# AiX-im/Sample-based-GNN

Hardware: AMD Instinct MI355X
Metric: sampled-edges/sec + epoch time, 2-hop GCN on Reddit-shaped graph @1/2/4/8 GPUs (higher is better)
Workload: dtype fp32 (GEMM inputs fp32, split exactly into three bf16 pieces in the kernels, 6 bf16 MFMA products, fp32 accumulate; aggregation fp32)

## Files before the change

### sample-based-gnn_amd/csrc/gemmx3.hip

```cpp
#include "mfma_lds.hpp"
#include <type_traits>

namespace nts_hip {


__device__ __forceinline__ f32x16 x3_mfma6(const bf16x8 (&a)[3], const bf16x8 (&b)[3], f32x16 acc) {
  acc = __builtin_amdgcn_mfma_f32_32x32x16_bf16(a[2], b[0], acc, 0, 0, 0);
  acc = __builtin_amdgcn_mfma_f32_32x32x16_bf16(a[1], b[1], acc, 0, 0, 0);
  acc = __builtin_amdgcn_mfma_f32_32x32x16_bf16(a[0], b[2], acc, 0, 0, 0);
  acc = __builtin_amdgcn_mfma_f32_32x32x16_bf16(a[1], b[0], acc, 0, 0, 0);
  acc = __builtin_amdgcn_mfma_f32_32x32x16_bf16(a[0], b[1], acc, 0, 0, 0);
  acc = __builtin_amdgcn_mfma_f32_32x32x16_bf16(a[0], b[0], acc, 0, 0, 0);
  return acc;
}

constexpr int kX3Threads = 512;
constexpr int kX3BRaw = 16 * 512;
constexpr int kX3BPl = 16 * 256;



template <int TPW, int PR, bool BM = false>
__global__ __launch_bounds__(kX3Threads, 1) void k_x3_tn(int M, int K, const float* __restrict__ X,
                                                        uint64_t ldx, const uint32_t* __restrict__ amap,
                                                        const float* __restrict__ B, uint64_t ldb,
                                                        float* __restrict__ C, uint64_t ldc, int kchunk,
                                                        uint64_t split_stride, int nnb,
                                                        const float* __restrict__ Xm, uint64_t ldxm,
                                                        float bscale) {
  static_assert(2 * PR <= 6, "X DMA pieces per wave and step");
  extern __shared__ __attribute__((aligned(16))) char x3tn[];
  const int Kp = (M + 31) / 32 * 32, RB = 4 * Kp, RW = Kp;
  const int xstage = 16 * RB;
  char* const sx = x3tn;
  char* const sbr = sx + 3 * xstage;
  char* const sbp = sbr + 2 * kX3BRaw;
  char* const sbm = sbp + 6 * kX3BPl;
  uint32_t* const sid = reinterpret_cast<uint32_t*>(sbm + (BM ? 2 * kX3BRaw : 0));
  const int tid = threadIdx.x, lane = tid & 63;
  const int wv = __builtin_amdgcn_readfirstlane(tid >> 6);
  const int nb = blockIdx.x % nnb, split = blockIdx.x / nnb;
  const int n0 = nb * 128;
  const int kbeg = split * kchunk, kend = min(K, kbeg + kchunk), klast = kend - kbeg - 1;
  if (klast < 0) return;
  const int nsteps = (kend - kbeg + 15) / 16;
  for (int k = tid; k < 16 * (nsteps + 3); k += kX3Threads)
    sid[k] = amap ? amap[kbeg + min(k, klast)] : (uint32_t)(kbeg + min(k, klast));
  __syncthreads();
  const uint32_t lsx = lds_addr(sx), lsbr = lds_addr(sbr), lsbm = lds_addr(sbm);
  auto ids_read = [&](int s) { return *reinterpret_cast<const uint2*>(sid + 16 * s + 2 * wv); };
  auto ids_uni = [&](uint2 u) {
    return make_uint2(__builtin_amdgcn_readfirstlane(u.x), __builtin_amdgcn_readfirstlane(u.y));
  };
  auto issue_x1 = [&](int s, uint2 id, int q) {
    const int row = 2 * wv + q / PR, part = q % PR;
    const int off = 1024 * part + 16 * lane;
    const char* src = reinterpret_cast<const char*>(X + (uint64_t)(q < PR ? id.x : id.y) * ldx) + off;
    const uint32_t dst = __builtin_amdgcn_readfirstlane(lsx + (s % 3) * xstage + row * RB + 1024 * part);
    if (off < RB) glds16(src, dst);
  };
  auto issue_b = [&](int s) {
    const int row = 2 * wv + (lane >> 5);
    const int k = kbeg + min(16 * s + row, klast);
    glds16(B + (uint64_t)k * ldb + n0 + 4 * (lane & 31), lsbr + (s & 1) * kX3BRaw + 1024 * wv);
    if constexpr (BM)
      glds16(Xm + (uint64_t)k * ldxm + n0 + 4 * (lane & 31), lsbm + (s & 1) * kX3BRaw + 1024 * wv);
  };
  const int sr = tid >> 5, sc = 4 * (tid & 31);
  const int soff = tr_off(sr, sc / 8) + 8 * ((sc / 4) & 1);
  auto splitb_read = [&](int s) {
    float4 v = *reinterpret_cast<const float4*>(sbr + (s & 1) * kX3BRaw + 512 * sr + 4 * sc);
    if constexpr (BM) {
      const float4 m = *reinterpret_cast<const float4*>(sbm + (s & 1) * kX3BRaw + 512 * sr + 4 * sc);
      v.x = m.x > 0.f ? v.x * bscale : 0.f;
      v.y = m.y > 0.f ? v.y * bscale : 0.f;
      v.z = m.z > 0.f ? v.z * bscale : 0.f;
      v.w = m.w > 0.f ? v.w * bscale : 0.f;
    }
    return v;
  };
  auto splitb_write = [&](int s, float4 v) {
    const bool ok = 16 * s + sr <= klast;
    uint32_t q0[2], q1[2], q2[2];
    split3_pair(ok ? v.x : 0.f, ok ? v.y : 0.f, q0[0], q1[0], q2[0]);
    split3_pair(ok ? v.z : 0.f, ok ? v.w : 0.f, q0[1], q1[1], q2[1]);
    char* dst = sbp + (s & 1) * 3 * kX3BPl + soff;
    *reinterpret_cast<uint2*>(dst) = make_uint2(q0[0], q0[1]);
    *reinterpret_cast<uint2*>(dst + kX3BPl) = make_uint2(q1[0], q1[1]);
    *reinterpret_cast<uint2*>(dst + 2 * kX3BPl) = make_uint2(q2[0], q2[1]);
  };
  const int wn = wv & 1, wm = wv >> 1;
  const int T32 = (M + 31) / 32;
  const int m_lo = wm * T32 / 4, nmt = (wm + 1) * T32 / 4 - m_lo;
  const int c = lane & 31, h = lane >> 5;
  const int half = (lane >> 4) & 1, tq = (lane & 15) >> 2, tp = lane & 3;
  int boff[2][2];
#pragma unroll
  for (int nt = 0; nt < 2; ++nt) {
    const int ch = (2 * (64 * wn + 32 * nt + 16 * half + 4 * tp)) / 16;
    boff[nt][0] = tr_off(8 * h + tq, ch) + 8 * (tp & 1);
    boff[nt][1] = tr_off(8 * h + tq + 4, ch) + 8 * (tp & 1);
  }
  int xcol[TPW];
#pragma unroll
  for (int t = 0; t < TPW; ++t) xcol[t] = 32 * max(0, min(m_lo + min(t, nmt - 1), T32 - 1)) + 8 * h * RW + c;
  f32x16 acc[TPW][2];
#pragma unroll
  for (int t = 0; t < TPW; ++t)
#pragma unroll
    for (int nt = 0; nt < 2; ++nt)
#pragma unroll
      for (int v = 0; v < 16; ++v) acc[t][nt][v] = 0.f;
  issue_b(0);
  asm volatile("s_waitcnt vmcnt(0)" ::: "memory");
  raw_barrier();
  splitb_write(0, splitb_read(0));
  issue_b(1);
  {
    const uint2 i0 = ids_uni(ids_read(0)), i1 = ids_uni(ids_read(1));
#pragma unroll
    for (int q = 0; q < 2 * PR; ++q) issue_x1(0, i0, q);
#pragma unroll
    for (int q = 0; q < 2 * PR; ++q) issue_x1(1, i1, q);
  }
  uint2 idn = ids_uni(ids_read(2));
  for (int s = 0; s < nsteps; ++s) {
    asm volatile("s_waitcnt vmcnt(0)" ::: "memory");
    raw_barrier();
    issue_b(s + 2);
    const char* pl = sbp + (s & 1) * 3 * kX3BPl;
    bf16x8 bq[2][3];
#pragma unroll
    for (int nt = 0; nt < 2; ++nt)
#pragma unroll
      for (int p = 0; p < 3; ++p) {
        const s16x4 lo = __builtin_amdgcn_ds_read_tr16_b64_v4i16((lds_s16x4*)(pl + p * kX3BPl + boff[nt][0]));
        const s16x4 hi = __builtin_amdgcn_ds_read_tr16_b64_v4i16((lds_s16x4*)(pl + p * kX3BPl + boff[nt][1]));
        const s16x8 w = {lo[0], lo[1], lo[2], lo[3], hi[0], hi[1], hi[2], hi[3]};
        bq[nt][p] = __builtin_bit_cast(bf16x8, w);
      }
    const float* xs = reinterpret_cast<const float*>(sx + (s % 3) * xstage);
    float xr[2][8];
    uint32_t ap[2][3][4];
    auto rd = [&](int t, int j) { return xs[xcol[t] + j * RW]; };
    auto sp = [&](int t, int jp) {
      split3_pair(xr[t & 1][2 * jp], xr[t & 1][2 * jp + 1], ap[t & 1][0][jp], ap[t & 1][1][jp],
                ap[t & 1][2][jp]);
    };
#pragma unroll
    for (int j = 0; j < 8; ++j) xr[0][j] = rd(0, j);
    if constexpr (TPW > 1) {
#pragma unroll
      for (int j = 0; j < 8; ++j) xr[1][j] = rd(1, j);
    }
#pragma unroll
    for (int jp = 0; jp < 4; ++jp) sp(0, jp);
    const uint2 idx = idn;
    float4 bv = make_float4(0.f, 0.f, 0.f, 0.f);
    uint2 idr = make_uint2(0u, 0u);
#pragma unroll
    for (int t = 0; t < TPW; ++t) {
      bf16x8 a[3];
#pragma unroll
      for (int p = 0; p < 3; ++p)
        a[p] = __builtin_bit_cast(bf16x8, (u32x4){ap[t & 1][p][0], ap[t & 1][p][1], ap[t & 1][p][2], ap[t & 1][p][3]});
#pragma unroll
      for (int k = 0; k < 12; ++k) {
        __builtin_amdgcn_sched_barrier(0);
        {
          const int nt = k & 1, pr = k >> 1;
          const int pa = pr == 0 ? 2 : pr == 1 ? 1 : pr == 2 ? 0 : pr == 3 ? 1 : 0;
          const int pb = pr == 0 ? 0 : pr == 1 ? 1 : pr == 2 ? 2 : pr == 3 ? 0 : pr == 4 ? 1 : 0;
          acc[t][nt] = __builtin_amdgcn_mfma_f32_32x32x16_bf16(a[pa], bq[nt][pb], acc[t][nt], 0, 0, 0);
        }
        if (t + 2 < TPW && k < 8) xr[t & 1][k] = rd(t + 2, k);
        if (t + 1 < TPW && (k == 3 || k == 5 || k == 7 || k == 9)) sp(t + 1, (k - 3) / 2);
        if (t == 0 && (k & 1) && k / 2 < 2 * PR) issue_x1(s + 2, idx, k / 2);
        constexpr int tB = TPW >= 2 ? 1 : 0, kBr = TPW >= 2 ? 1 : 5, kBw = TPW >= 2 ? 8 : 9;
        constexpr int tI = TPW >= 3 ? 2 : 0, kIr = TPW >= 3 ? 1 : 6, kIw = TPW >= 3 ? 10 : 11;
        if (t == tB && k == kBr) bv = splitb_read(s + 1);
        if (t == tB && k == kBw) splitb_write(s + 1, bv);
        if (t == tI && k == kIr) idr = ids_read(s + 3);
        if (t == tI && k == kIw) idn = ids_uni(idr);
      }
      __builtin_amdgcn_sched_barrier(0);
    }
  }
  asm volatile("s_waitcnt vmcnt(0)" ::: "memory");
  raw_barrier();
  float* Cb = C + (uint64_t)split * split_stride;
#pragma unroll
  for (int nt = 0; nt < 2; ++nt) {
    const int col = n0 + 64 * wn + 32 * nt + c;
#pragma unroll
    for (int t = 0; t < TPW; ++t) {
      if (t >= nmt) continue;
#pragma unroll
      for (int v = 0; v < 16; ++v) {
        const int row = 32 * (m_lo + t) + 8 * (v / 4) + 4 * h + (v % 4);
        if (row < M) Cb[(uint64_t)row * ldc + col] = acc[t][nt][v];
      }
    }
  }
}

constexpr int kX3NnImg = 8 * 3 * 1024;
constexpr int kX3NnAWave = 2 * 2048;
constexpr int kX3NnA = 8 * kX3NnAWave;
constexpr int kX3NnLds = 2 * kX3NnImg + 3 * kX3NnA;
struct X3Epi {
  uint32_t keep_threshold = 0;
  float scale = 1.f;
  uint64_t seed = 0, offset = 0;
};


template <bool EPI>
__global__ __launch_bounds__(kX3Threads, 1) void k_x3_nn(int M, int N, int K, const float* __restrict__ X,
                                                        uint64_t ldx, const uint32_t* __restrict__ amap,
                                                        const char* __restrict__ bimg,
                                                        float* __restrict__ C, uint64_t ldc, int rounds,
                                                        X3Epi ep) {
  extern __shared__ __attribute__((aligned(16))) char x3nn[];
  char* const sb = x3nn;
  char* const sa = x3nn + 2 * kX3NnImg;
  const int tid = threadIdx.x, lane = tid & 63;
  const int wv = __builtin_amdgcn_readfirstlane(tid >> 6);
  const int i = lane & 15, q = lane >> 4;
  const int nb = blockIdx.y, n0 = nb * 128;
  const int T = (M + 15) / 16;
  const int64_t Wn = (int64_t)gridDim.x * 8, gw = (int64_t)blockIdx.x * 8 + wv;
  const int t_lo = (int)(gw * T / Wn), t_hi = (int)((gw + 1) * T / Wn);
  const int nsteps = (K + 31) / 32;
  const size_t bstride = (size_t)gridDim.y * kX3NnImg;
  const uint32_t lsb = lds_addr(sb), lsa = lds_addr(sa);
  const char* bsrc = bimg + (size_t)nb * kX3NnImg + wv * 1024 + 16 * lane;
  const int gr = (lane >> 1) & 15, gpo = 8 * (lane >> 5) + 4 * (lane & 1);
  const float* arow[2];
  auto set_rows = [&](int rd) {
#pragma unroll
    for (int rt = 0; rt < 2; ++rt) {
      const int t = min(t_lo + 2 * rd + rt, T - 1);
      const int64_t row = (int64_t)t * 16 + gr;
      const uint64_t rr = (uint64_t)(row < M ? row : M - 1);
      arow[rt] = X + (amap ? (uint64_t)amap[rr] : rr) * ldx + gpo;
    }
  };
  auto issue_b = [&](int s) {
    const uint32_t dst = lsb + (s & 1) * kX3NnImg + wv * 1024;
    const char* src = bsrc + (size_t)s * bstride;
#pragma unroll
    for (int p = 0; p < 3; ++p) glds16(src + 8192 * p, dst + 8192 * p);
  };
  auto issue_a = [&](int s) {
    const uint32_t dst = lsa + (s % 3) * kX3NnA + wv * kX3NnAWave;
#pragma unroll
    for (int rt = 0; rt < 2; ++rt)
#pragma unroll
      for (int h = 0; h < 2; ++h) glds16(arow[rt] + 32 * s + 16 * h, dst + rt * 2048 + h * 1024);
  };
  f32x4 acc[2][8];
  float xr[2][8];
  uint32_t ap[2][2][3][4];
  auto read_a = [&](int s, int rt) {
    typedef float f4v __attribute__((ext_vector_type(4)));
    const char* as = sa + (s % 3) * kX3NnA + wv * kX3NnAWave + 32 * (i + 16 * q) + rt * 2048;
    const f4v u = *reinterpret_cast<const f4v*>(as);
    const f4v v = *reinterpret_cast<const f4v*>(as + 16);
    const float x[8] = {u[0], u[1], u[2], u[3], v[0], v[1], v[2], v[3]};
#pragma unroll
    for (int j = 0; j < 8; ++j) xr[rt][j] = x[j];
    if (32 * s + 32 > K) {
#pragma unroll
      for (int j = 0; j < 8; ++j) xr[rt][j] = 32 * s + 8 * q + j < K ? x[j] : 0.f;
    }
  };
  auto split_a = [&](auto par, int rt, int jp) {
    constexpr int P = decltype(par)::value;
    split3_pair(xr[rt][2 * jp], xr[rt][2 * jp + 1], ap[P][rt][0][jp], ap[P][rt][1][jp], ap[P][rt][2][jp]);
  };
  auto step = [&](int s, auto par, auto ntc) {
    constexpr int P = decltype(par)::value, NT = decltype(ntc)::value;
    if (s > 0) {
      asm volatile("s_waitcnt vmcnt(0)" ::: "memory");
      raw_barrier();
      if (s + 1 < nsteps) issue_b(s + 1);
      if (s + 2 < nsteps) issue_a(s + 2);
    }
    const char* img = sb + (s & 1) * kX3NnImg;
    auto getb = [&](int ct, int p) {
      return *reinterpret_cast<const bf16x8*>(img + ct * 3072 + p * 1024 + 16 * lane);
    };
    bf16x8 bf[2][3];
#pragma unroll
    for (int p = 0; p < 3; ++p) bf[0][p] = getb(0, p);
    bf16x8 a[2][3];
#pragma unroll
    for (int rt = 0; rt < NT; ++rt)
#pragma unroll
      for (int p = 0; p < 3; ++p)
        a[rt][p] = __builtin_bit_cast(bf16x8, (u32x4){ap[P][rt][p][0], ap[P][rt][p][1], ap[P][rt][p][2], ap[P][rt][p][3]});
#pragma unroll
    for (int ct = 0; ct < 8; ++ct) {
#pragma unroll
      for (int k = 0; k < 6 * NT; ++k) {
        __builtin_amdgcn_sched_barrier(0);
        {
          const int rt = NT == 2 ? (k & 1) : 0, pr = NT == 2 ? (k >> 1) : k;
          const int pa = pr == 0 ? 2 : pr == 1 ? 1 : pr == 2 ? 0 : pr == 3 ? 1 : 0;
          const int pb = pr == 0 ? 0 : pr == 1 ? 1 : pr == 2 ? 2 : pr == 3 ? 0 : pr == 4 ? 1 : 0;
          if constexpr (EPI)
            acc[rt][ct] = __builtin_amdgcn_mfma_f32_16x16x32_bf16(a[rt][pa], bf[ct & 1][pb], acc[rt][ct], 0, 0, 0);
          else
            acc[rt][ct] = __builtin_amdgcn_mfma_f32_16x16x32_bf16(bf[ct & 1][pb], a[rt][pa], acc[rt][ct], 0, 0, 0);
        }
        if (ct + 1 < 8 && (k == 0 || k == 2 || k == 4)) bf[(ct + 1) & 1][k / 2] = getb(ct + 1, k / 2);
        if (ct == 4 && k == 0) asm volatile("s_waitcnt vmcnt(0)" ::: "memory");
        if (ct == 4 && k == 1) read_a(s + 1, 0);
        if constexpr (NT == 2) {
          if (ct == 4 && k == 3) read_a(s + 1, 1);
          if ((ct == 5 || ct == 6) && k % 3 == 1) split_a(std::integral_constant<int, 1 - P>{}, ct - 5, k / 3);
        } else {
          if (ct == 5 && (k & 1)) split_a(std::integral_constant<int, 1 - P>{}, 0, k >> 1);
          if (ct == 6 && k == 1) split_a(std::integral_constant<int, 1 - P>{}, 0, 3);
        }
      }
      __builtin_amdgcn_sched_barrier(0);
    }
  };
  auto round_steps = [&](auto ntc) {
    constexpr int NT = decltype(ntc)::value;
    issue_b(0);
    issue_a(0);
    if (nsteps > 1) issue_a(1);
    asm volatile("s_waitcnt vmcnt(0)" ::: "memory");
    raw_barrier();
    if (nsteps > 1) issue_b(1);
    if (nsteps > 2) issue_a(2);
#pragma unroll
    for (int rt = 0; rt < NT; ++rt) read_a(0, rt);
#pragma unroll
    for (int rt = 0; rt < NT; ++rt)
#pragma unroll
      for (int jp = 0; jp < 4; ++jp) split_a(std::integral_constant<int, 0>{}, rt, jp);
    for (int s = 0; s < nsteps; s += 2) {
      step(s, std::integral_constant<int, 0>{}, ntc);
      if (s + 1 < nsteps) step(s + 1, std::integral_constant<int, 1>{}, ntc);
    }
  };
  for (int rd = 0; rd < rounds; ++rd) {
    const int nt = min(2, max(0, t_hi - (t_lo + 2 * rd)));
    set_rows(rd);
#pragma unroll
    for (int rt = 0; rt < 2; ++rt)
#pragma unroll
      for (int ct = 0; ct < 8; ++ct) acc[rt][ct] = f32x4{0.f, 0.f, 0.f, 0.f};
    if (nt == 2) round_steps(std::integral_constant<int, 2>{});
    else round_steps(std::integral_constant<int, 1>{});
    raw_barrier();
    if constexpr (!EPI) {
#pragma unroll
      for (int rt = 0; rt < 2; ++rt) {
        if (rt >= nt) continue;
        const int64_t row = (int64_t)(t_lo + 2 * rd + rt) * 16 + i;
        if (row >= M) continue;
#pragma unroll
        for (int ct = 0; ct < 8; ++ct) {
          const int col = n0 + 16 * ct + 4 * q;
          if (col >= N) continue;
          float* dst = C + (uint64_t)row * ldc + col;
          if (ldc % 4 == 0 && (uintptr_t)C % 16 == 0)
            *reinterpret_cast<f32x4*>(dst) = acc[rt][ct];
          else
#pragma unroll
            for (int v = 0; v < 4; ++v) dst[v] = acc[rt][ct][v];
        }
      }
      continue;
    }
#pragma unroll
    for (int rt = 0; rt < 2; ++rt) {
      if (rt >= nt) continue;
      const int64_t r4 = (int64_t)(t_lo + 2 * rd + rt) * 16 + 4 * q;
#pragma unroll
      for (int ct = 0; ct < 8; ++ct) {
        const uint32_t col = (uint32_t)(n0 + 16 * ct + i);
        if ((int)col >= N) continue;
        float o[4] = {acc[rt][ct][0], acc[rt][ct][1], acc[rt][ct][2], acc[rt][ct][3]};
        if constexpr (EPI) {
          const uint4 rnd = dropout_words((uint64_t)r4, col, ep.seed, ep.offset);
          const uint32_t wd[4] = {rnd.x, rnd.y, rnd.z, rnd.w};
#pragma unroll
          for (int v = 0; v < 4; ++v)
            o[v] = (dropout_bits(wd[v], col) >= ep.keep_threshold && o[v] > 0.f) ? o[v] * ep.scale : 0.f;
        }
#pragma unroll
        for (int v = 0; v < 4; ++v)
          if (r4 + v < M) C[(uint64_t)(r4 + v) * ldc + col] = o[v];
      }
    }
  }
}

constexpr int kX3N7Threads = 256;
constexpr int kX3N7RT = 7;
constexpr int kX3N7Lds = 3 * kX3NnImg;
__device__ constexpr int kX3N7Pb[kX3N7RT] = {0, 1, 2, 0, 1, 2, 1};

template <int B, int E, class F>
__device__ __forceinline__ void x3_sfor(F&& f) {
  if constexpr (B < E) {
    f(std::integral_constant<int, B>{});
    x3_sfor<B + 1, E>(f);
  }
}

template <int O>
__device__ __forceinline__ void x3_split_op(const float (&x)[8], float (&r)[8], float (&f)[8],
                                            uint32_t (&p)[3][4]) {
  auto pk = [](float a, float b) {
    return __builtin_bit_cast(uint32_t, __builtin_convertvector((f32x2){a, b}, bf16x2));
  };
  if constexpr (O < 4) {
    p[0][O] = pk(x[2 * O], x[2 * O + 1]);
  } else if constexpr (O < 12) {
    constexpr int e = O - 4;
    f[e] = __uint_as_float((e & 1) ? (p[0][e / 2] & 0xffff0000u) : (p[0][e / 2] << 16));
  } else if constexpr (O < 20) {
    r[O - 12] = x[O - 12] - f[O - 12];
  } else if constexpr (O < 24) {
    p[1][O - 20] = pk(r[2 * (O - 20)], r[2 * (O - 20) + 1]);
  } else if constexpr (O < 32) {
    constexpr int e = O - 24;
    f[e] = __uint_as_float((e & 1) ? (p[1][e / 2] & 0xffff0000u) : (p[1][e / 2] << 16));
  } else if constexpr (O < 40) {
    r[O - 32] = r[O - 32] - f[O - 32];
  } else if constexpr (O < 44) {
    p[2][O - 40] = pk(r[2 * (O - 40)], r[2 * (O - 40) + 1]);
  }
}

constexpr int kX3N7Bq = 1;
template <int RT, bool EPI = false>
__global__ __launch_bounds__(kX3N7Threads, 1) void k_x3_nn7(int M, int N, int K, const float* __restrict__ X,
                                                           uint64_t ldx, const uint32_t* __restrict__ amap,
                                                           const char* __restrict__ bimg, float* __restrict__ C,
                                                           uint64_t ldc, int rounds, X3Epi ep) {
  static_assert(RT == kX3N7RT, "the W piece schedule is written for 7 tiles");
  extern __shared__ __attribute__((aligned(16))) char x3n7[];
  const int tid = threadIdx.x, lane = tid & 63;
  const int wv = __builtin_amdgcn_readfirstlane(tid >> 6);
  const int i = lane & 15, q = lane >> 4;
  const int nb = blockIdx.y, n0 = nb * 128;
  const int T = (M + 15) / 16;
  const int64_t Wn = (int64_t)gridDim.x * 4, gw = (int64_t)blockIdx.x * 4 + wv;
  const int t_lo = (int)(gw * T / Wn), t_hi = (int)((gw + 1) * T / Wn);
  const int nsteps = (K + 31) / 32;
  const uint64_t bstride = (uint64_t)gridDim.y * kX3NnImg;
  const uint32_t lsw = lds_addr(x3n7) + 6144 * wv;
  const char* bsrc = bimg + (size_t)nb * kX3NnImg + 6144 * wv + 16 * lane;
  auto row_id = [&](int rd, int rt) -> uint32_t {
    int t = min(t_lo + RT * rd + rt, max(t_hi, t_lo + 1) - 1);
    t = min(t, T - 1);
    int64_t r = (int64_t)t * 16 + i;
    if (r >= M) r = M - 1;
    return amap ? amap[r] : (uint32_t)r;
  };
  const float* ptr[RT];
  uint32_t nid[RT];
#pragma unroll
  for (int rt = 0; rt < RT; ++rt) ptr[rt] = X + (uint64_t)row_id(0, rt) * ldx + 8 * q;
#pragma unroll
  for (int rt = 0; rt < RT; ++rt) nid[rt] = row_id(1, rt);
  f32x4 wst[6];
  char* const wdst = x3n7 + 6144 * wv + 16 * lane;
  auto load_w = [&](int s, auto pc) {
    constexpr int piece = decltype(pc)::value;
    wst[piece] = *reinterpret_cast<const f32x4*>(bsrc + (size_t)s * bstride + 1024 * piece);
  };
  const uint32_t wdst_l = lds_addr(wdst);
  auto store_w = [&](int buf, auto pc) {
    constexpr int piece = decltype(pc)::value;
    const uint32_t addr = wdst_l + buf * kX3NnImg;
    const f32x4 v = wst[piece];
    asm volatile("ds_write_b128 %0, %1 offset:%2" ::"v"(addr), "v"(v), "n"(1024 * piece) : "memory");
  };
  float4 raw[RT][2];
  auto load_a = [&](int rt, int s) {
    const float* p = ptr[rt] + 32 * s;
    raw[rt][0] = *reinterpret_cast<const float4*>(p);
    raw[rt][1] = *reinterpret_cast<const float4*>(p + 4);
  };
  f32x4 acc[RT][8];
#pragma unroll
  for (int rt = 0; rt < RT; ++rt)
#pragma unroll
    for (int ct = 0; ct < 8; ++ct) acc[rt][ct] = f32x4{0.f, 0.f, 0.f, 0.f};
  uint32_t pcs[3][3][4];
  constexpr int NB = kX3N7Bq + 1;
  bf16x8 bq[NB][3];
  float sr[8], sf[8];
  auto read_b = [&](int buf, int ct, int p) {
    return *reinterpret_cast<const bf16x8*>(x3n7 + buf * kX3NnImg + ct * 3072 + p * 1024 + 16 * lane);
  };
  auto mask_k = [&](float (&x)[8], int s) {
    if (32 * s + 32 > K) {
#pragma unroll
      for (int j = 0; j < 8; ++j) x[j] = 32 * s + 8 * q + j < K ? x[j] : 0.f;
    }
  };
  auto raw8 = [&](int rt, float (&x)[8]) {
    x[0] = raw[rt][0].x; x[1] = raw[rt][0].y; x[2] = raw[rt][0].z; x[3] = raw[rt][0].w;
    x[4] = raw[rt][1].x; x[5] = raw[rt][1].y; x[6] = raw[rt][1].z; x[7] = raw[rt][1].w;
  };
  x3_sfor<0, 6>([&](auto pc) {
    load_w(0, pc);
    store_w(0, pc);
  });
#pragma unroll
  for (int rt = 0; rt < RT; ++rt) load_a(rt, 0);
  asm volatile("s_waitcnt vmcnt(0)" ::: "memory");
  raw_barrier();
  {
    float x[8];
    raw8(0, x);
    mask_k(x, 0);
#pragma unroll
    for (int j = 0; j < 4; ++j) split3_pair(x[2 * j], x[2 * j + 1], pcs[0][0][j], pcs[0][1][j], pcs[0][2][j]);
  }
  load_a(0, 1);
#pragma unroll
  for (int c = 0; c < kX3N7Bq; ++c)
#pragma unroll
    for (int p = 0; p < 3; ++p) bq[c][p] = read_b(0, c, p);
  int wb = 0;
  for (int rd = 0; rd < rounds; ++rd) {
  for (int s = 0; s < nsteps; ++s) {
    int s1 = s + 1, rd1 = rd;
    if (s1 == nsteps) { s1 = 0; ++rd1; }
    int s2 = s1 + 1, rd2 = rd1;
    if (s2 == nsteps) { s2 = 0; ++rd2; }
    const int wb1 = wb == 2 ? 0 : wb + 1;
    x3_sfor<0, RT>([&](auto rtc) {
      constexpr int rt = decltype(rtc)::value;
      constexpr int cur = kX3N7Pb[rt], nxt = kX3N7Pb[rt + 1 < RT ? rt + 1 : 0];
      bf16x8 a[3];
#pragma unroll
      for (int p = 0; p < 3; ++p)
        a[p] = __builtin_bit_cast(bf16x8, (u32x4){pcs[cur][p][0], pcs[cur][p][1], pcs[cur][p][2], pcs[cur][p][3]});
      constexpr int srt = rt + 1 < RT ? rt + 1 : 0;
      const int ss = rt + 1 < RT ? s : s1;
      float x[8];
      if constexpr (rt + 1 == RT) {
        x3_sfor<0, 6>([&](auto pc) { store_w(wb1, pc); });
        asm volatile("s_waitcnt lgkmcnt(0)" ::: "memory");
        raw_barrier();
      }
      __builtin_amdgcn_sched_barrier(0);
      raw8(srt, x);
      mask_k(x, ss);
      x3_sfor<0, 48>([&](auto kc) {
        constexpr int k = decltype(kc)::value;
        constexpr int ct = k / 6, pr = k % 6;
        __builtin_amdgcn_sched_barrier(0);
        {
          constexpr int pa = pr == 0 ? 2 : pr == 1 ? 1 : pr == 2 ? 0 : pr == 3 ? 1 : 0;
          constexpr int pb = pr == 0 ? 0 : pr == 1 ? 1 : pr == 2 ? 2 : pr == 3 ? 0 : pr == 4 ? 1 : 0;
          if constexpr (EPI)
            acc[rt][ct] = __builtin_amdgcn_mfma_f32_16x16x32_bf16(a[pa], bq[ct % NB][pb], acc[rt][ct], 0, 0, 0);
          else
            acc[rt][ct] = __builtin_amdgcn_mfma_f32_16x16x32_bf16(bq[ct % NB][pb], a[pa], acc[rt][ct], 0, 0, 0);
        }
        if constexpr (pr < 3) {
          constexpr int cn = ct + kX3N7Bq;
          if constexpr (cn < 8) bq[cn % NB][pr] = read_b(wb, cn, pr);
          else if constexpr (rt + 1 < RT) bq[(cn - 8) % NB][pr] = read_b(wb, cn - 8, pr);
          else bq[(cn - 8) % NB][pr] = read_b(wb1, cn - 8, pr);
        }
        if constexpr (k >= 1 && k <= 44) x3_split_op<k - 1>(x, sr, sf, pcs[nxt]);
        if constexpr (rt + 1 < RT) {
          if constexpr (rt == 0 && k >= 2 && k < 8)
            load_w(s1, std::integral_constant<int, (k >= 2 && k < 8 ? k - 2 : 0)>{});
        }
        if constexpr (k == 22) {
          if constexpr (rt + 1 < RT) {
            if (s1 == 0 && rd1 < rounds) ptr[srt] = X + (uint64_t)nid[srt] * ldx + 8 * q;
            load_a(srt, s1);
          } else {
            if (s2 == 0 && rd2 < rounds) ptr[0] = X + (uint64_t)nid[0] * ldx + 8 * q;
            load_a(0, s2);
          }
        }
      });
      __builtin_amdgcn_sched_barrier(0);
    });
    wb = wb1;
  }
    {
      x3_sfor<0, RT>([&](auto rtc) {
        constexpr int rt = decltype(rtc)::value;
        const int t = t_lo + RT * rd + rt;
        if constexpr (!EPI) {
          const int64_t row = (int64_t)t * 16 + i;
          if (t < t_hi && row < M) {
#pragma unroll
            for (int ct = 0; ct < 8; ++ct) {
              const int col = n0 + 16 * ct + 4 * q;
              if (col < N) *reinterpret_cast<f32x4*>(C + (uint64_t)row * ldc + col) = acc[rt][ct];
            }
          }
        } else if (t < t_hi) {
          const int64_t r4 = (int64_t)t * 16 + 4 * q;
          x3_sfor<0, 8>([&](auto ctc) {
            constexpr int ct = decltype(ctc)::value;
            const uint32_t col = (uint32_t)(n0 + 16 * ct + i);
            if ((int)col < N) {
              const uint4 rnd = dropout_words((uint64_t)r4, col, ep.seed, ep.offset);
              const uint32_t wd[4] = {rnd.x, rnd.y, rnd.z, rnd.w};
              x3_sfor<0, 4>([&](auto vc) {
                constexpr int v = decltype(vc)::value;
                const float o = acc[rt][ct][v];
                if (r4 + v < M)
                  C[(uint64_t)(r4 + v) * ldc + col] =
                      (dropout_bits(wd[v], col) >= ep.keep_threshold && o > 0.f) ? o * ep.scale : 0.f;
              });
            }
          });
        }
#pragma unroll
        for (int ct = 0; ct < 8; ++ct) acc[rt][ct] = f32x4{0.f, 0.f, 0.f, 0.f};
      });
#pragma unroll
      for (int rt = 0; rt < RT; ++rt) nid[rt] = row_id(rd + 2, rt);
    }
  }
  asm volatile("s_waitcnt vmcnt(0)" ::: "memory");
}


bool x3_tn_ok(int M, int N, int K, const float* A, uint64_t lda, const float* B, uint64_t ldb,
              const float* Xm, uint64_t ldxm) {
  const int Kp = (M + 31) / 32 * 32;
  const int lds = 3 * 16 * 4 * Kp + 2 * kX3BRaw + 6 * kX3BPl + (Xm ? 2 * kX3BRaw : 0) + 4 * 16 * 3 +
                  4 * 256;
  return M >= 32 && lds <= 160 * 1024 && N % 128 == 0 && K >= 256 && lda >= (uint64_t)Kp && lda % 4 == 0 &&
         (uintptr_t)A % 16 == 0 && ldb % 4 == 0 && (uintptr_t)B % 16 == 0 &&
         (!Xm || (ldxm % 4 == 0 && (uintptr_t)Xm % 16 == 0));
}

int x3_tn(nts_hip_ctx* ctx, int M, int N, int K, const float* A, uint64_t lda, const uint32_t* amap,
          const float* B, uint64_t ldb, float* C, uint64_t ldc, const float* Xm, uint64_t ldxm,
          float bscale) {
  const int Kp = (M + 31) / 32 * 32, RB = 4 * Kp;
  const int nnb = N / 128;
  const int ksteps = (K + 15) / 16;
  int splits = std::max(1, std::min(256 / nnb, ksteps / 8));
  int kchunk = ((ksteps + splits - 1) / splits) * 16;
  const int fixed = 3 * 16 * RB + 2 * kX3BRaw + 6 * kX3BPl + (Xm ? 2 * kX3BRaw : 0) + 4 * 16 * 3;
  kchunk = std::min(kchunk, (160 * 1024 - fixed) / 4 / 16 * 16);
  splits = (K + kchunk - 1) / kchunk;
  const int lds = fixed + 4 * kchunk;
  const uint64_t stride = (uint64_t)M * N;
  float* out = C;
  uint64_t ldo = ldc;
  if (splits > 1) {
    NTS_RET(ensure_scratch(ctx, stride * splits * sizeof(float) + 256));
    out = (float*)ctx->scratch;
    ldo = N;
  }
  const int pr = (RB + 1023) / 1024;
  const int tpw = ((M + 31) / 32 + 3) / 4;
#define NTS_X3TN(T, P, BMK)                                                                      \
  do {                                                                                           \
    NTS_HIP_TRY(hipFuncSetAttribute(reinterpret_cast<const void*>(&k_x3_tn<T, P, BMK>),         \
                                    hipFuncAttributeMaxDynamicSharedMemorySize, lds));           \
    hipLaunchKernelGGL((k_x3_tn<T, P, BMK>), dim3(nnb * splits), dim3(kX3Threads), lds,         \
                       ctx->stream, M, K, A, lda, amap, B, ldb, out, ldo, kchunk,                \
                       splits > 1 ? stride : (uint64_t)0, nnb, Xm, ldxm, bscale);                \
  } while (0)
  if (Xm && tpw <= 1 && pr == 1) {
    NTS_X3TN(1, 1, true);
  } else if (Xm) {
    return NTS_ERR_INVALID;
  } else if (pr == 1) NTS_X3TN(5, 1, false);
  else if (pr == 2) NTS_X3TN(5, 2, false);
  else NTS_X3TN(5, 3, false);
#undef NTS_X3TN
  NTS_LAUNCH_CHECK();
  if (splits == 1) return NTS_OK;
  return sum_splits(ctx->stream, out, splits, stride, M, N, C, ldc);
}

bool x3_tn_bm_ok(int M, int N, int K, const float* A, uint64_t lda, const float* B, uint64_t ldb,
                 const float* Xm, uint64_t ldxm) {
  return M <= 128 && x3_tn_ok(M, N, K, A, lda, B, ldb, Xm, ldxm);
}

bool x3_nn_ok(int M, int N, int K, const float* A, uint64_t lda) {
  const int Kp = (K + 31) / 32 * 32;
  return M >= 256 && K >= 1 && N % 16 == 0 && lda >= (uint64_t)Kp && lda % 4 == 0 &&
         (uintptr_t)A % 16 == 0;
}
bool x3_nn7_ok(int M, int N, int K, const float* A, uint64_t lda) {
  return x3_nn_ok(M, N, K, A, lda) && (K + 31) / 32 >= 4 && M >= 32768;
}

int x3_nn(nts_hip_ctx* ctx, bool epi, int M, int N, int K, const float* A, uint64_t lda,
          const uint32_t* amap, const char* bimg, float* C, uint64_t ldc, uint32_t keep_threshold,
          float scale, uint64_t seed, uint64_t offset) {
  X3Epi ep;
  ep.keep_threshold = keep_threshold;
  ep.scale = scale;
  ep.seed = seed;
  ep.offset = offset;
  const int ncb = (N + 127) / 128;
  const int T = (M + 15) / 16;
  int gx = std::max(8, (256 / ncb) / 8 * 8);
  gx = std::min(gx, std::max(8, ((T + 15) / 16 + 7) / 8 * 8));
  const int64_t Wn = (int64_t)gx * 8;
  const int max_tiles = (int)((T + Wn - 1) / Wn);
  const int rounds = (max_tiles + 1) / 2;
  const dim3 grid(gx, ncb);
#define NTS_X3NN(E)                                                                            \
  do {                                                                                         \
    NTS_HIP_TRY(hipFuncSetAttribute(reinterpret_cast<const void*>(&k_x3_nn<E>),                \
                                    hipFuncAttributeMaxDynamicSharedMemorySize, kX3NnLds));    \
    hipLaunchKernelGGL((k_x3_nn<E>), grid, dim3(kX3Threads), kX3NnLds, ctx->stream, M, N, K, A, \
                       lda, amap, bimg, C, ldc, rounds, ep);                                   \
  } while (0)
  const bool c16 = ldc % 4 == 0 && (uintptr_t)C % 16 == 0;
  if (x3_nn7_ok(M, N, K, A, lda) && (epi || c16)) {
    const int T7 = (M + 15) / 16;
    const int gx7 = std::max(1, std::min(std::max(1, 256 / ncb), (T7 + 4 * kX3N7RT - 1) / (4 * kX3N7RT)));
    const int64_t W7 = (int64_t)gx7 * 4;
    const int tiles7 = (int)((T7 + W7 - 1) / W7);
    const int rounds7 = (tiles7 + kX3N7RT - 1) / kX3N7RT;
#define NTS_X3N7(E)                                                                              \
  do {                                                                                           \
    NTS_HIP_TRY(hipFuncSetAttribute(reinterpret_cast<const void*>(&k_x3_nn7<kX3N7RT, E>),        \
                                    hipFuncAttributeMaxDynamicSharedMemorySize, kX3N7Lds));      \
    hipLaunchKernelGGL((k_x3_nn7<kX3N7RT, E>), dim3(gx7, ncb), dim3(kX3N7Threads), kX3N7Lds,     \
                       ctx->stream, M, N, K, A, lda, amap, bimg, C, ldc, rounds7, ep);           \
  } while (0)
    if (epi) NTS_X3N7(true);
    else NTS_X3N7(false);
#undef NTS_X3N7
    NTS_LAUNCH_CHECK();
    return NTS_OK;
  }
  if (epi) NTS_X3NN(true);
  else NTS_X3NN(false);
#undef NTS_X3NN
  NTS_LAUNCH_CHECK();
  return NTS_OK;
}

}
```

Baseline: 1.918 billion.

## Repartition TN x3 GEMM wave tiles so each A fragment feeds full 128-column width

Wave pairs that previously split the N dimension (64 columns each) over the same M tiles now split the M tiles between them. Each wave computes full 128-column tiles, reusing each split A fragment across four accumulators, and one leftover tile is shared as before. This halves per-wave A-row LDS reads and bf16 splitting, but every wave must now load B fragments for both column halves. Those extra B reads are prefetched and interleaved into the MFMA sequence. The cost is higher accumulator and register pressure and more complex scheduling.

```diff
diff --git a/sample-based-gnn_amd/csrc/gemmx3.hip b/sample-based-gnn_amd/csrc/gemmx3.hip
--- a/sample-based-gnn_amd/csrc/gemmx3.hip
+++ b/sample-based-gnn_amd/csrc/gemmx3.hip
@@ -92,25 +92,37 @@
   const int wn = wv & 1, wm = wv >> 1;
   const int T32 = (M + 31) / 32;
   const int m_lo = wm * T32 / 4, nmt = (wm + 1) * T32 / 4 - m_lo;
+  constexpr int FS = TPW / 2, FA = FS ? FS : 1;
+  const int full = nmt / 2;
+  const bool shared = nmt & 1;
+  const int f_lo = m_lo + wn * (full + (nmt & 1));
   const int c = lane & 31, h = lane >> 5;
   const int half = (lane >> 4) & 1, tq = (lane & 15) >> 2, tp = lane & 3;
-  int boff[2][2];
-#pragma unroll
-  for (int nt = 0; nt < 2; ++nt) {
-    const int ch = (2 * (64 * wn + 32 * nt + 16 * half + 4 * tp)) / 16;
-    boff[nt][0] = tr_off(8 * h + tq, ch) + 8 * (tp & 1);
-    boff[nt][1] = tr_off(8 * h + tq + 4, ch) + 8 * (tp & 1);
-  }
-  int xcol[TPW];
-#pragma unroll
-  for (int t = 0; t < TPW; ++t) xcol[t] = 32 * max(0, min(m_lo + min(t, nmt - 1), T32 - 1)) + 8 * h * RW + c;
-  f32x16 acc[TPW][2];
-#pragma unroll
-  for (int t = 0; t < TPW; ++t)
-#pragma unroll
-    for (int nt = 0; nt < 2; ++nt)
-#pragma unroll
-      for (int v = 0; v < 16; ++v) acc[t][nt][v] = 0.f;
+  int boff[2][2][2];
+#pragma unroll
+  for (int hf = 0; hf < 2; ++hf)
+#pragma unroll
+    for (int nt = 0; nt < 2; ++nt) {
+      const int ch = (2 * (64 * (wn ^ hf) + 32 * nt + 16 * half + 4 * tp)) / 16;
+      boff[hf][nt][0] = tr_off(8 * h + tq, ch) + 8 * (tp & 1);
+      boff[hf][nt][1] = tr_off(8 * h + tq + 4, ch) + 8 * (tp & 1);
+    }
+  int xcol[FS + 1];
+#pragma unroll
+  for (int f = 0; f < FS; ++f) xcol[f] = 32 * max(0, min(f_lo + min(f, full - 1), T32 - 1)) + 8 * h * RW + c;
+  xcol[FS] = 32 * max(0, min(m_lo + full, T32 - 1)) + 8 * h * RW + c;
+  f32x16 acc[FA][4];
+  f32x16 accs[2];
+#pragma unroll
+  for (int f = 0; f < FS; ++f)
+#pragma unroll
+    for (int q = 0; q < 4; ++q)
+#pragma unroll
+      for (int v = 0; v < 16; ++v) acc[f][q][v] = 0.f;
+#pragma unroll
+  for (int nt = 0; nt < 2; ++nt)
+#pragma unroll
+    for (int v = 0; v < 16; ++v) accs[nt][v] = 0.f;
   issue_b(0);
   asm volatile("s_waitcnt vmcnt(0)" ::: "memory");
   raw_barrier();
@@ -129,41 +141,66 @@
     raw_barrier();
     issue_b(s + 2);
     const char* pl = sbp + (s & 1) * 3 * kX3BPl;
-    bf16x8 bq[2][3];
+    bf16x8 bq[2][2][3];
+    auto rdb = [&](int hf, int nt, int p) {
+      const s16x4 lo = __builtin_amdgcn_ds_read_tr16_b64_v4i16((lds_s16x4*)(pl + p * kX3BPl + boff[hf][nt][0]));
+      const s16x4 hi = __builtin_amdgcn_ds_read_tr16_b64_v4i16((lds_s16x4*)(pl + p * kX3BPl + boff[hf][nt][1]));
+      const s16x8 w = {lo[0], lo[1], lo[2], lo[3], hi[0], hi[1], hi[2], hi[3]};
+      bq[hf][nt][p] = __builtin_bit_cast(bf16x8, w);
+    };
 #pragma unroll
     for (int nt = 0; nt < 2; ++nt)
 #pragma unroll
-      for (int p = 0; p < 3; ++p) {
-        const s16x4 lo = __builtin_amdgcn_ds_read_tr16_b64_v4i16((lds_s16x4*)(pl + p * kX3BPl + boff[nt][0]));
-        const s16x4 hi = __builtin_amdgcn_ds_read_tr16_b64_v4i16((lds_s16x4*)(pl + p * kX3BPl + boff[nt][1]));
-        const s16x8 w = {lo[0], lo[1], lo[2], lo[3], hi[0], hi[1], hi[2], hi[3]};
-        bq[nt][p] = __builtin_bit_cast(bf16x8, w);
-      }
+      for (int p = 0; p < 3; ++p) rdb(0, nt, p);
     const float* xs = reinterpret_cast<const float*>(sx + (s % 3) * xstage);
-    float xr[2][8];
+    float xr[8];
     uint32_t ap[2][3][4];
-    auto rd = [&](int t, int j) { return xs[xcol[t] + j * RW]; };
-    auto sp = [&](int t, int jp) {
-      split3_pair(xr[t & 1][2 * jp], xr[t & 1][2 * jp + 1], ap[t & 1][0][jp], ap[t & 1][1][jp],
-                ap[t & 1][2][jp]);
+    auto rd = [&](int i, int j) { return xs[xcol[i] + j * RW]; };
+    auto sp = [&](int i, int jp) {
+      split3_pair(xr[2 * jp], xr[2 * jp + 1], ap[i & 1][0][jp], ap[i & 1][1][jp], ap[i & 1][2][jp]);
     };
 #pragma unroll
-    for (int j = 0; j < 8; ++j) xr[0][j] = rd(0, j);
-    if constexpr (TPW > 1) {
-#pragma unroll
-      for (int j = 0; j < 8; ++j) xr[1][j] = rd(1, j);
-    }
+    for (int j = 0; j < 8; ++j) xr[j] = rd(0, j);
 #pragma unroll
     for (int jp = 0; jp < 4; ++jp) sp(0, jp);
     const uint2 idx = idn;
     float4 bv = make_float4(0.f, 0.f, 0.f, 0.f);
     uint2 idr = make_uint2(0u, 0u);
 #pragma unroll
-    for (int t = 0; t < TPW; ++t) {
+    for (int f = 0; f < FS; ++f) {
       bf16x8 a[3];
 #pragma unroll
       for (int p = 0; p < 3; ++p)
-        a[p] = __builtin_bit_cast(bf16x8, (u32x4){ap[t & 1][p][0], ap[t & 1][p][1], ap[t & 1][p][2], ap[t & 1][p][3]});
+        a[p] = __builtin_bit_cast(bf16x8, (u32x4){ap[f & 1][p][0], ap[f & 1][p][1], ap[f & 1][p][2], ap[f & 1][p][3]});
+#pragma unroll
+      for (int k = 0; k < 24; ++k) {
+        __builtin_amdgcn_sched_barrier(0);
+        const int kk = k % 12, hf = (k / 12) ^ (f & 1);
+        {
+          const int nt = kk & 1, pr = kk >> 1;
+          const int pa = pr == 0 ? 2 : pr == 1 ? 1 : pr == 2 ? 0 : pr == 3 ? 1 : 0;
+          const int pb = pr == 0 ? 0 : pr == 1 ? 1 : pr == 2 ? 2 : pr == 3 ? 0 : pr == 4 ? 1 : 0;
+          acc[f][2 * hf + nt] =
+              __builtin_amdgcn_mfma_f32_32x32x16_bf16(a[pa], bq[hf][nt][pb], acc[f][2 * hf + nt], 0, 0, 0);
+        }
+        if (k < 8) xr[k] = rd(f + 1, k);
+        if (k == 10 || k == 13 || k == 16 || k == 19) sp(f + 1, (k - 10) / 3);
+        const int g = 2 * f + k / 12;
+        const int hn = g + 1 == 2 * FS ? 0 : ((g + 1) & 1) ^ (((g + 1) >> 1) & 1);
+        if (hn != hf && kk >= 6) rdb(hn, kk & 1, kk < 8 ? 0 : kk < 10 ? 2 : 1);
+        if (f == 0 && (k & 1) && k / 2 < 2 * PR) issue_x1(s + 2, idx, k / 2);
+        if (f == 0 && k == 9) bv = splitb_read(s + 1);
+        if (f == 0 && k == 12) splitb_write(s + 1, bv);
+        if (f == 0 && k == 14) idr = ids_read(s + 3);
+        if (f == 0 && k == 22) idn = ids_uni(idr);
+      }
+      __builtin_amdgcn_sched_barrier(0);
+    }
+    if (FS == 0 || shared) {
+      bf16x8 a[3];
+#pragma unroll
+      for (int p = 0; p < 3; ++p)
+        a[p] = __builtin_bit_cast(bf16x8, (u32x4){ap[FS & 1][p][0], ap[FS & 1][p][1], ap[FS & 1][p][2], ap[FS & 1][p][3]});
 #pragma unroll
       for (int k = 0; k < 12; ++k) {
         __builtin_amdgcn_sched_barrier(0);
@@ -171,17 +208,15 @@
           const int nt = k & 1, pr = k >> 1;
           const int pa = pr == 0 ? 2 : pr == 1 ? 1 : pr == 2 ? 0 : pr == 3 ? 1 : 0;
           const int pb = pr == 0 ? 0 : pr == 1 ? 1 : pr == 2 ? 2 : pr == 3 ? 0 : pr == 4 ? 1 : 0;
-          acc[t][nt] = __builtin_amdgcn_mfma_f32_32x32x16_bf16(a[pa], bq[nt][pb], acc[t][nt], 0, 0, 0);
-        }
-        if (t + 2 < TPW && k < 8) xr[t & 1][k] = rd(t + 2, k);
-        if (t + 1 < TPW && (k == 3 || k == 5 || k == 7 || k == 9)) sp(t + 1, (k - 3) / 2);
-        if (t == 0 && (k & 1) && k / 2 < 2 * PR) issue_x1(s + 2, idx, k / 2);
-        constexpr int tB = TPW >= 2 ? 1 : 0, kBr = TPW >= 2 ? 1 : 5, kBw = TPW >= 2 ? 8 : 9;
-        constexpr int tI = TPW >= 3 ? 2 : 0, kIr = TPW >= 3 ? 1 : 6, kIw = TPW >= 3 ? 10 : 11;
-        if (t == tB && k == kBr) bv = splitb_read(s + 1);
-        if (t == tB && k == kBw) splitb_write(s + 1, bv);
-        if (t == tI && k == kIr) idr = ids_read(s + 3);
-        if (t == tI && k == kIw) idn = ids_uni(idr);
+          accs[nt] = __builtin_amdgcn_mfma_f32_32x32x16_bf16(a[pa], bq[0][nt][pb], accs[nt], 0, 0, 0);
+        }
+        if constexpr (FS == 0) {
+          if ((k & 1) && k / 2 < 2 * PR) issue_x1(s + 2, idx, k / 2);
+          if (k == 5) bv = splitb_read(s + 1);
+          if (k == 9) splitb_write(s + 1, bv);
+          if (k == 6) idr = ids_read(s + 3);
+          if (k == 11) idn = ids_uni(idr);
+        }
       }
       __builtin_amdgcn_sched_barrier(0);
     }
@@ -190,15 +225,26 @@
   raw_barrier();
   float* Cb = C + (uint64_t)split * split_stride;
 #pragma unroll
-  for (int nt = 0; nt < 2; ++nt) {
-    const int col = n0 + 64 * wn + 32 * nt + c;
-#pragma unroll
-    for (int t = 0; t < TPW; ++t) {
-      if (t >= nmt) continue;
+  for (int q = 0; q < 4; ++q) {
+    const int col = n0 + 64 * (wn ^ (q >> 1)) + 32 * (q & 1) + c;
+#pragma unroll
+    for (int f = 0; f < FS; ++f) {
+      if (f >= full) continue;
 #pragma unroll
       for (int v = 0; v < 16; ++v) {
-        const int row = 32 * (m_lo + t) + 8 * (v / 4) + 4 * h + (v % 4);
-        if (row < M) Cb[(uint64_t)row * ldc + col] = acc[t][nt][v];
+        const int row = 32 * (f_lo + f) + 8 * (v / 4) + 4 * h + (v % 4);
+        if (row < M) Cb[(uint64_t)row * ldc + col] = acc[f][q][v];
+      }
+    }
+  }
+  if (shared) {
+#pragma unroll
+    for (int nt = 0; nt < 2; ++nt) {
+      const int col = n0 + 64 * wn + 32 * nt + c;
+#pragma unroll
+      for (int v = 0; v < 16; ++v) {
+        const int row = 32 * (m_lo + full) + 8 * (v / 4) + 4 * h + (v % 4);
+        if (row < M) Cb[(uint64_t)row * ldc + col] = accs[nt][v];
       }
     }
   }
```

Result: faster. 1.942 billion (median of 4 runs) (+1.3%).
